# PKU-EPIC/PartManip

Measured on AMD Instinct MI355X. Metric: PPO env-steps/sec (whole node), 4096 envs x 1024-pt clouds, higher is better.
Workload: dtype f32

## Files before the change

### include/partmanip_hip.h

```cpp
#ifndef PARTMANIP_HIP_H
#define PARTMANIP_HIP_H

#include <stddef.h>
#include <stdint.h>

#ifdef __cplusplus
extern "C" {
#endif

#define PM_OK 0
#define PM_EINVAL (-1)
#define PM_EWORKSPACE (-2)
#define PM_EALIGN (-3)
#define PM_EUNSUPPORTED (-4)

#define PM_ACT_NONE 0
#define PM_ACT_TANH 1
#define PM_ACT_RELU 2
#define PM_ACT_LRELU 3
#define PM_ACT_ELU 4
#define PM_ACT_SELU 5
#define PM_ACT_SIGMOID 6
#define PM_ACT_MAX 6

// ... 37 lines not shown
    const float* dY; long lddy; const float* W; long ldw; const float* H; long ldh; float* dX; long lddx; int M, N, K, act;
} pm_linear_bwd_data_desc;
typedef struct pm_linear_bwd_weight_desc {
    const float* dY; long lddy; const float* X; long ldx; float* dW; long lddw; float* db; long slab_stride; int M, N, K;
    int dy_cols, x_cols;
    int pad_;
} pm_linear_bwd_weight_desc;
int pm_linear_fwd_group_f32(int n, const pm_linear_fwd_desc* d, void* stream);
int pm_linear_bwd_data_group_f32(int n, const pm_linear_bwd_data_desc* d, void* stream);
int pm_linear_bwd_weight_group_f32(int n, const pm_linear_bwd_weight_desc* d, int splits, void* stream);
#define PM_LINEAR_PATH_SKINNY 0
#define PM_LINEAR_PATH_REG 1
#define PM_LINEAR_PATH_DMA 2
typedef struct pm_linear_variant {
    int path;
    int tm, tn;
    int lay;
    int stages;
    int vec;
    int big;
    int grid;
    int n;
    int vecC[PM_LINEAR_GROUP_MAX];
    int splits[PM_LINEAR_GROUP_MAX];
    int kchunk[PM_LINEAR_GROUP_MAX];
} pm_linear_variant;
int pm_linear_fwd_variant_f32(const float* X, long ldx, const float* W, long ldw, const float* b, const float* Y, long ldy,
                              int M, int N, int K, int act, pm_linear_variant* out);
int pm_linear_bwd_data_variant_f32(const float* dY, long lddy, const float* W, long ldw, const float* H, long ldh,
                                   const float* dX, long lddx, int M, int N, int K, int act, pm_linear_variant* out);
int pm_linear_bwd_weight_variant_f32(const float* dY, long lddy, const float* X, long ldx, const float* dW, long lddw,
                                     const float* db, int M, int N, int K, const void* workspace, pm_linear_variant* out);
int pm_linear_fwd_group_variant_f32(int n, const pm_linear_fwd_desc* d, pm_linear_variant* out);
int pm_linear_bwd_data_group_variant_f32(int n, const pm_linear_bwd_data_desc* d, pm_linear_variant* out);
int pm_linear_bwd_weight_group_variant_f32(int n, const pm_linear_bwd_weight_desc* d, int splits, pm_linear_variant* out);
size_t pm_linear_chain_workspace_bytes(int M);
int pm_linear_fwd_chain_f32(int n, const pm_linear_fwd_desc* d, void* workspace, size_t workspace_bytes, void* stream);
int pm_linear_bwd_data_chain_f32(int n, const pm_linear_bwd_data_desc* d, void* workspace, size_t workspace_bytes, void* stream);

size_t pm_pointnet_packed_elems(void);
int pm_pointnet_pack_weights_f32(const float* W2, const float* W3, float* packed, void* stream);
int pm_pointnet_enc_fwd_f32(const float* x, long ldx, int B, int P, int C, int sub_mean, const float* W1,
                            const float* b1, const float* b2, const float* b3, const float* packed,
                            int max_mean, float* feat, long ldf, int32_t* argmax,
                            float* h2_save ,
                            int act ,
                            void* stream);
size_t pm_pointnet_packed_screen_bytes(void);
int pm_pointnet_pack_weights_screen(const float* W3, const float* b3, void* packed, void* stream);
int pm_pointnet_enc_fwd_screen_f32(const float* x, long ldx, int B, int P, int C, int sub_mean, const float* W1,
                                   const float* b1, const float* b2, const float* b3, const float* packed,
                                   const void* packed_screen, int max_mean, float* feat, long ldf, int32_t* argmax,
                                   float* h2_save, unsigned long long* counters, void* stream);
size_t pm_pointnet_packed_bf3_bytes(void);
int pm_pointnet_pack_weights_bf3(const float* W2, const float* W3, void* packed, void* stream);
int pm_pointnet_enc_fwd_bf3(const float* x, long ldx, int B, int P, int C, int sub_mean, const float* W1,
                            const float* b1, const float* b2, const float* b3, const void* packed, int max_mean,
                            float* feat, long ldf, int32_t* argmax, float* h2_save ,
                            void* stream);
size_t pm_pointnet_packed_bf6_bytes(void);
int pm_pointnet_pack_weights_bf6(const float* W2, const float* W3, void* packed, void* stream);
int pm_pointnet_enc_fwd_bf6(const float* x, long ldx, int B, int P, int C, int sub_mean, const float* W1,
                            const float* b1, const float* b2, const float* b3, const void* packed, int max_mean,
                            float* feat, long ldf, int32_t* argmax, float* h2_save ,
                            void* stream);
size_t pm_pointnet_enc_bwd_workspace_bytes(int B, int P, int C);
int pm_pointnet_enc_bwd_f32(const float* x, long ldx, int B, int P, int C, int sub_mean, const float* W1,
                            const float* b1, const float* b2, const float* W3, const float* packed,
                            int max_mean, const float* dfeat, long ldf, const int32_t* argmax, float* dW1,
                            float* db1, float* dW2, float* db2, float* dW3, float* db3,
                            const float* h2_saved ,
                            int act , void* workspace, size_t workspace_bytes, void* stream);
size_t pm_pointnet_packed_bwd_bf6_bytes(void);
int pm_pointnet_pack_weights_bwd_bf6(const float* W2, void* packed, void* stream);
int pm_pointnet_enc_bwd_bf6(const float* x, long ldx, int B, int P, int C, int sub_mean, const float* W1,
                            const float* b1, const float* b2, const float* W3, const float* packed,
                            const void* packed_w2_bf6, int max_mean, const float* dfeat, long ldf, const int32_t* argmax,
                            float* dW1, float* db1, float* dW2, float* db2, float* dW3, float* db3, const float* h2_saved,
                            void* workspace, size_t workspace_bytes, void* stream);

int pm_ppo_actor_loss_fwd_bwd_f32(const float* mu, long ldmu, const float* log_std, const float* actions,
                                  long lda, const float* old_logp, const float* adv, const float* old_mu,
                                  long ldom, const float* old_sigma, long ldos, int B, int A, float max_action,
                                  int act_tanh, float eps_clip, float desired_kl, const double* adv_moments,
                                  double adv_count, float* scal_out, float* dmu, long lddmu, float* dlog_std,
                                  void* workspace, size_t workspace_bytes, void* stream);
size_t pm_ppo_actor_loss_workspace_bytes(int B);
int pm_ppo_actor_head_supported(const float* H, long ldh, const float* W, long ldw, int A, int K, const float* dH, long lddh);
int pm_ppo_actor_head_f32(const float* H, long ldh, const float* W, long ldw, const float* bias, int K, int hidden_act,
                          const float* log_std, const float* actions, long lda, const float* old_logp, const float* adv,
                          const float* old_mu, long ldom, const float* old_sigma, long ldos, int B, int A, float max_action,
                          int act_tanh, float eps_clip, float desired_kl, const double* adv_moments, double adv_count,
                          float* scal_out, float* mu_out, long ldmu, float* dmu, long lddmu, float* dH, long lddh,
                          float* dlog_std, void* workspace, size_t workspace_bytes, unsigned int* counter, void* stream);
int pm_gaussian_logp_f32(const float* mu, long ldmu, const float* log_std, const float* actions, long lda,
                         int B, int A, float max_action, int act_tanh, float* logp, float* entropy,
                         void* stream);

int pm_value_loss_fwd_bwd_f32(const float* V, const float* returns, const float* old_values, int B,
                              int clipped, float eps_clip, const float* clip_mean_extern, float grad_scale,
                              float* scal_out, float* dV, long lddv, void* stream);

size_t pm_value_head_workspace_bytes(void);
int pm_value_head_supported(const float* H, long ldh, const float* W, int K, const float* dH, long lddh);
int pm_value_head_f32(const float* H, long ldh, const float* W, const float* bias, int K, int hidden_act, const float* returns,
                      const float* old_values, int B, int clipped, float eps_clip, const float* clip_mean_extern,
// ... 297 lines not shown
```

### partmanip_amd/_lib.py

```python
import ctypes as C
import os

import torch

HERE = os.path.dirname(os.path.abspath(__file__))
LIB_PATH = os.environ.get("PARTMANIP_HIP_LIB") or os.path.join(HERE, "lib", "libpartmanip_hip.so")

P, I, L, F, D, Z = C.c_void_p, C.c_int, C.c_long, C.c_float, C.c_double, C.c_size_t

SIGNATURES = {
    "pm_version": (I, []),
    "pm_gae_scan_f32": (I, [P, P, P, P, P, P, P, I, I, F, F, I, F, P]),
    "pm_moments_workspace_bytes": (Z, [L]),
    "pm_moments_f64": (I, [P, L, P, P, Z, P]),
    "pm_normalize_apply_f32": (I, [P, L, P, D, F, P]),
    "pm_gather_rows_f32": (I, [P, P, P, L, L, L, L, P]),
    "pm_linear_fwd_f32": (I, [P, L, P, L, P, P, L, I, I, I, I, P]),
    "pm_linear_bwd_data_f32": (I, [P, L, P, L, P, L, P, L, I, I, I, I, P]),
    "pm_linear_bwd_weight_workspace_bytes": (Z, [I, I, I]),
    "pm_linear_bwd_weight_f32": (I, [P, L, P, L, P, L, P, I, I, I, P, Z, P]),
    "pm_linear_fwd_group_f32": (I, [I, P, P]),
    "pm_linear_bwd_data_group_f32": (I, [I, P, P]),
    "pm_linear_chain_workspace_bytes": (C.c_size_t, [I]),
    "pm_linear_fwd_chain_f32": (I, [I, P, P, C.c_size_t, P]),
    "pm_linear_bwd_data_chain_f32": (I, [I, P, P, C.c_size_t, P]),
    "pm_linear_bwd_weight_group_f32": (I, [I, P, I, P]),
    "pm_linear_fwd_variant_f32": (I, [P, L, P, L, P, P, L, I, I, I, I, P]),
    "pm_linear_bwd_data_variant_f32": (I, [P, L, P, L, P, L, P, L, I, I, I, I, P]),
    "pm_linear_bwd_weight_variant_f32": (I, [P, L, P, L, P, L, P, I, I, I, P, P]),
    "pm_linear_fwd_group_variant_f32": (I, [I, P, P]),
    "pm_linear_bwd_data_group_variant_f32": (I, [I, P, P]),
    "pm_linear_bwd_weight_group_variant_f32": (I, [I, P, I, P]),
    "pm_clip_adam_group_f32": (I, [I, P, P]),
    "pm_grad_slab_sum_f32": (I, [P, P, L, L, I, P]),
    "pm_pointnet_packed_elems": (Z, []),
    "pm_pointnet_pack_weights_f32": (I, [P, P, P, P]),
    "pm_pointnet_enc_fwd_f32": (I, [P, L, I, I, I, I, P, P, P, P, P, I, P, L, P, P, I, P]),
    "pm_pointnet_packed_screen_bytes": (Z, []),
    "pm_pointnet_pack_weights_screen": (I, [P, P, P, P]),
    "pm_pointnet_enc_fwd_screen_f32": (I, [P, L, I, I, I, I, P, P, P, P, P, P, I, P, L, P, P, P, P]),
    "pm_pointnet_packed_bf3_bytes": (Z, []),
    "pm_pointnet_pack_weights_bf3": (I, [P, P, P, P]),
    "pm_pointnet_enc_fwd_bf3": (I, [P, L, I, I, I, I, P, P, P, P, P, I, P, L, P, P, P]),
    "pm_pointnet_packed_bf6_bytes": (Z, []),
    "pm_pointnet_pack_weights_bf6": (I, [P, P, P, P]),
    "pm_pointnet_enc_fwd_bf6": (I, [P, L, I, I, I, I, P, P, P, P, P, I, P, L, P, P, P]),
    "pm_pointnet_enc_bwd_workspace_bytes": (Z, [I, I, I]),
    "pm_pointnet_enc_bwd_f32": (I, [P, L, I, I, I, I, P, P, P, P, P, I, P, L, P, P, P, P, P, P, P, P, I, P, Z, P]),
    "pm_pointnet_packed_bwd_bf6_bytes": (Z, []),
    "pm_pointnet_pack_weights_bwd_bf6": (I, [P, P, P]),
    "pm_pointnet_enc_bwd_bf6": (I, [P, L, I, I, I, I, P, P, P, P, P, P, I, P, L, P, P, P, P, P, P, P, P, P, Z, P]),
    "pm_ppo_actor_loss_fwd_bwd_f32": (I, [P, L, P, P, L, P, P, P, L, P, L, I, I, F, I, F, F, P, D, P, P, L, P, P, Z, P]),
    "pm_ppo_actor_loss_workspace_bytes": (Z, [I]),
    "pm_ppo_actor_head_supported": (I, [P, L, P, L, I, I, P, L]),
    "pm_ppo_actor_head_f32": (I, [P, L, P, L, P, I, I, P, P, L, P, P, P, L, P, L, I, I, F, I, F, F, P, D, P, P, L, P, L, P, L, P, P, Z, P, P]),
    "pm_gaussian_logp_f32": (I, [P, L, P, P, L, I, I, F, I, P, P, P]),
    "pm_gaussian_logp_bwd_f32": (I, [P, L, P, P, L, I, I, F, I, P, P, P, L, P, P]),
    "pm_action_activation_bwd_f32": (I, [P, P, P, L, F, I, P]),
    "pm_value_loss_fwd_bwd_f32": (I, [P, P, P, I, I, F, P, F, P, P, L, P]),
    "pm_value_head_workspace_bytes": (Z, []),
    "pm_value_head_supported": (I, [P, L, P, I, P, L]),
    "pm_value_head_f32": (I, [P, L, P, P, I, I, P, P, I, I, F, P, F, P, P, P, L, P, L, P, Z, P, P]),
    "pm_mse_tanh_loss_fwd_bwd_f32": (I, [P, L, P, L, I, I, F, I, F, P, P, L, P]),
    "pm_action_activation_f32": (I, [P, P, L, F, I, P]),
    "pm_clip_adam_workspace_bytes": (Z, [L]),
    "pm_clip_adam_step_f32": (I, [P, P, P, P, L, L, F, D, D, D, D, P, P, P, P, Z, P]),
    "pm_ppo_accumulate_stats_f32": (I, [P, P, I, P]),
    "pm_fps_workspace_bytes": (Z, [I, I]),
    "pm_fps_f32": (I, [P, I, I, I, I, P, P, Z, P]),
    "pm_ball_query_f32": (I, [P, P, I, I, I, F, I, P, P]),
    "pm_group_points_f32": (I, [P, P, I, I, I, I, I, P, P]),
    "pm_group_points_bwd_f32": (I, [P, P, I, I, I, I, I, P, P]),
    "pm_group_concat_f32": (I, [P, P, P, P, I, I, I, I, I, I, P, P]),
    "pm_group_concat_bwd_f32": (I, [P, P, I, I, I, I, I, I, P, P]),
    "pm_maxpool_rows_f32": (I, [P, L, I, I, P, L, P, P]),
    "pm_maxpool_rows_bwd_f32": (I, [P, L, P, L, I, I, P, P, P]),
    "pm_depth_backproject_f32": (I, [P, I, I, I, I, P, F, F, F, F, P, P, P, P]),
    "pm_depth_compact_f32": (I, [P, I, I, P, P, P]),
    "pm_fps_varlen_f32": (I, [P, I, I, I, I, P, I, P, P, Z, P]),
    "pm_fps_varlen_workspace_bytes": (Z, [I, I]),
    "pm_tsdf_select_f32": (I, [P, I, I, F, F, P, P, P]),
    "pm_gaussian_sample_f32": (I, [P, L, P, P, I, I, F, I, P, P, P, P]),
    "pm_rms_update_workspace_bytes": (Z, [I]),
    "pm_rms_update_f32": (I, [P, L, I, I, I, P, P, P, P, Z, P]),
    "pm_rms_normalize_f32": (I, [P, L, I, I, P, P, P, L, P]),
    "pm_rms_moments_f64": (I, [P, L, I, I, P, P, Z, P]),
    "pm_rms_apply_moments_f32": (I, [P, L, I, I, P, P, P, P]),
    "pm_tsdf_sparse_gather_f32": (I, [P, P, P, I, I, I, P, P]),
    "pm_im2col3d_f32": (I, [P, I, I, I, I, I, I, I, I, L, L, L, L, L, P, I, P]),
    "pm_conv3d_c1_supported": (I, [I, I]),
    "pm_conv3d_c1_wgrad_workspace_bytes": (Z, [I]),
    "pm_conv3d_c1_fwd_f32": (I, [P, I, I, I, I, I, I, I, L, L, L, L, P, P, I, I, P, L, P, P]),
    "pm_conv3d_c1_wgrad_f32": (I, [P, L, P, I, I, I, I, I, I, I, L, L, L, L, I, P, L, P, P, P, Z, P]),
# ... 139 lines not shown
```

### partmanip_amd/algo_utils/network.py

```python
import math
from typing import NamedTuple, Optional

import torch
import torch.nn as nn

from .. import ops

_LINEAR_ACT = {"tanh": ops.ACT_TANH, "relu": ops.ACT_RELU, "crelu": ops.ACT_RELU, "lrelu": ops.ACT_LRELU, "elu": ops.ACT_ELU,
               "selu": ops.ACT_SELU, "sigmoid": ops.ACT_SIGMOID}
_SUPPORTED_ACT = {"tanh": ops.ACT_TANH}
import os as _os
CHAIN_LAUNCH = _os.environ.get("PARTMANIP_CHAIN", "0") == "1"
PN_SCREEN_DEFAULT = True


def get_activation(act_name):
    table = {"elu": nn.ELU, "selu": nn.SELU, "relu": nn.ReLU, "crelu": nn.ReLU, "lrelu": nn.LeakyReLU,
             "tanh": nn.Tanh, "sigmoid": nn.Sigmoid}
    if act_name not in table:
        print("invalid activation function!")
        return None
    return table[act_name]()


# ... 199 lines not shown
        for g, m in zip(gains, lins):
            torch.nn.init.orthogonal_(m.weight, gain=g)
        object.__setattr__(self, "_chain", _LinearChain(lins, _act_code(net_cfg['activation'], linear_only=True)))

    def set_grad_views(self, views):
        idx = [i for i, m in enumerate(self.model) if isinstance(m, nn.Linear)]
        self._chain.grads = [(views[f"model.{i}.weight"], views[f"model.{i}.bias"]) for i in idx]

    def hip_forward(self, x, out=None, x_w=None):
        return self._chain.forward(x, out, x_w)

    def hip_backward(self, dy):
        self._chain.backward(dy, self._workspace(dy.device))


class PointNet(_HipNet):

    def __init__(self, input_dim, output_dim, net_cfg, proprio_shape):
        super().__init__()
        self.max_mean_concat = net_cfg['max_mean']
        self.point_num = int(net_cfg.get('point_num', 1024))
        act = net_cfg['activation']
        self.mlp = nn.Sequential(
            nn.Linear(input_dim // self.point_num, 128), get_activation(act),
            nn.Linear(128, 256), get_activation(act),
            nn.Linear(256, 512),
        )
        self.final_mlp = nn.Sequential(
            nn.Linear(512 * (1 + self.max_mean_concat) + proprio_shape, 128), get_activation(act),
            nn.Linear(128, 32), get_activation(act),
            nn.Linear(32, output_dim),
        )
        self.proprio_shape = proprio_shape
        self.substract_mean = net_cfg['sub_mean']
        self.count = 0
        self.in_channels = input_dim // self.point_num
        self.feat_dim = 512 * (1 + int(self.max_mean_concat))
        self.precision = net_cfg.get('precision', 'f32')
        self.save_h2 = bool(net_cfg.get('save_h2', True))
        if self.precision not in ('f32', 'bf16x3', 'bf16x6'):
            raise ValueError(f"PointNet precision '{self.precision}'")
        self.precision_bwd = net_cfg.get('precision_bwd', 'f32')
        if self.precision_bwd not in ('f32', 'bf16x6'):
            raise ValueError(f"PointNet precision_bwd '{self.precision_bwd}'")
        if self.precision_bwd != 'f32' and not self.save_h2:
            raise ValueError("PointNet precision_bwd 'bf16x6' reads the forward's saved layer 2 (save_h2: True)")
        code = _act_code(act, linear_only=True)
        if (self.precision != 'f32' or self.precision_bwd != 'f32') and code != ops.ACT_TANH:
            raise NotImplementedError(f"PointNet precision '{self.precision}' / precision_bwd '{self.precision_bwd}' is a tanh "
                                      f"kernel; activation '{act}' runs on 'f32'")
        screen = _os.environ.get("PARTMANIP_PN_SCREEN")
        self.screen = bool(net_cfg.get('screen', PN_SCREEN_DEFAULT)) if screen is None else screen == "1"
        self.screen_counters = None
        object.__setattr__(self, "_act", code)
        object.__setattr__(self, "_packed_s", None)
        object.__setattr__(self, "_head", _LinearChain([self.final_mlp[0], self.final_mlp[2], self.final_mlp[4]], code))
        object.__setattr__(self, "_enc_grads", None)
        object.__setattr__(self, "_packed", None)
        object.__setattr__(self, "_packed3", None)
        object.__setattr__(self, "_packed6", None)
        object.__setattr__(self, "_packed6b", None)

    def set_grad_views(self, views):
        self._head.grads = [(views[f"final_mlp.{i}.weight"], views[f"final_mlp.{i}.bias"]) for i in (0, 2, 4)]
        object.__setattr__(self, "_enc_grads", [views[f"mlp.{i}.{k}"] for i in (0, 2, 4) for k in ("weight", "bias")])

    def _pack(self, device):
        if self._packed is None or self._packed.device != device:
            object.__setattr__(self, "_packed", torch.empty(ops.pointnet_packed_elems(), device=device))
        ops.pointnet_pack(self.mlp[2].weight.data, self.mlp[4].weight.data, self._packed)
        return self._packed

    def forward(self, x):
        with torch.no_grad():
            return self.hip_forward(x, save_h2=False)

    def _h2_buffer(self, B, device):
        return self._scratch("_h2buf", B * self.point_num * 256, device).view(B, self.point_num, 256)

    def hip_forward(self, x, out=None, save_h2=None):
        B = x.shape[0]
        packed = self._pack(x.device)
        feat = torch.empty(B, self.feat_dim + self.proprio_shape, device=x.device)
        argmax = torch.empty(B, 512, dtype=torch.int32, device=x.device)
        save_h2 = self.save_h2 if save_h2 is None else save_h2
        h2 = self._h2_buffer(B, x.device) if save_h2 else None
        if self.precision == 'bf16x3':
            if self._packed3 is None or self._packed3.device != x.device:
                object.__setattr__(self, "_packed3", torch.empty(int(ops.lib.pm_pointnet_packed_bf3_bytes()),
                                                                 dtype=torch.uint8, device=x.device))
            ops.pointnet_pack_bf3(self.mlp[2].weight.data, self.mlp[4].weight.data, self._packed3)
            ops.pointnet_enc_fwd_bf3(x, self.point_num, self.in_channels, self.substract_mean, self.mlp[0].weight.data,
                                     self.mlp[0].bias.data, self.mlp[2].bias.data, self.mlp[4].bias.data,
                                     self._packed3, self.max_mean_concat, feat, argmax, h2)
        elif self.precision == 'bf16x6':
            if self._packed6 is None or self._packed6.device != x.device:
                object.__setattr__(self, "_packed6", torch.empty(int(ops.lib.pm_pointnet_packed_bf6_bytes()),
                                                                 dtype=torch.uint8, device=x.device))
            ops.pointnet_pack_bf6(self.mlp[2].weight.data, self.mlp[4].weight.data, self._packed6)
            ops.pointnet_enc_fwd_bf6(x, self.point_num, self.in_channels, self.substract_mean, self.mlp[0].weight.data,
                                     self.mlp[0].bias.data, self.mlp[2].bias.data, self.mlp[4].bias.data,
                                     self._packed6, self.max_mean_concat, feat, argmax, h2)
        elif self.screen and self._act == ops.ACT_TANH and self.point_num % 64 == 0:
            if self._packed_s is None or self._packed_s.device != x.device:
                object.__setattr__(self, "_packed_s", torch.empty(ops.pointnet_packed_screen_bytes(), dtype=torch.uint8,
                                                                  device=x.device))
            ops.pointnet_pack_screen(self.mlp[4].weight.data, self.mlp[4].bias.data, self._packed_s)
            ops.pointnet_enc_fwd_screen(x, self.point_num, self.in_channels, self.substract_mean, self.mlp[0].weight.data,
                                        self.mlp[0].bias.data, self.mlp[2].bias.data, self.mlp[4].bias.data, packed,
                                        self._packed_s, self.max_mean_concat, feat, argmax, h2, self.screen_counters)
        else:
            ops.pointnet_enc_fwd(x, self.point_num, self.in_channels, self.substract_mean, self.mlp[0].weight.data,
                                 self.mlp[0].bias.data, self.mlp[2].bias.data, self.mlp[4].bias.data, packed,
                                 self.max_mean_concat, feat, argmax, h2, self._act)
        if self.proprio_shape != 0:
            feat[:, self.feat_dim:].copy_(x[:, -self.proprio_shape:])
        object.__setattr__(self, "_saved", (x, feat, argmax, h2))
        return self._head.forward(feat, out)

    def hip_backward(self, dy):
        x, feat, argmax, h2 = self._saved
        ws = self._workspace(dy.device)
        dfeat = torch.empty_like(feat)
        self._head.backward(dy, ws, dx_out=dfeat)
        g = self._enc_grads
        if self.precision_bwd == 'bf16x6':
            if h2 is None:
                raise RuntimeError("PointNet precision_bwd 'bf16x6': the forward did not save layer 2 (an inference forward?)")
            if self._packed6b is None or self._packed6b.device != dy.device:
                object.__setattr__(self, "_packed6b", torch.empty(int(ops.lib.pm_pointnet_packed_bwd_bf6_bytes()),
                                                                  dtype=torch.uint8, device=dy.device))
            ops.pointnet_pack_bwd_bf6(self.mlp[2].weight.data, self._packed6b)
            ops.pointnet_enc_bwd_bf6(x, self.point_num, self.in_channels, self.substract_mean, self.mlp[0].weight.data,
                                     self.mlp[0].bias.data, self.mlp[2].bias.data, self.mlp[4].weight.data, self._packed,
                                     self._packed6b, self.max_mean_concat, dfeat, argmax, g[0], g[1], g[2], g[3], g[4], g[5],
                                     ws, h2)
            return
        ops.pointnet_enc_bwd(x, self.point_num, self.in_channels, self.substract_mean, self.mlp[0].weight.data,
                             self.mlp[0].bias.data, self.mlp[2].bias.data, self.mlp[4].weight.data, self._packed,
                             self.max_mean_concat, dfeat, argmax, g[0], g[1], g[2], g[3], g[4], g[5], ws, h2, self._act)


def _pad4(n):
    return (n + 3) // 4 * 4


class _GeomTabs(list):

    def __init__(self, it=()):
        super().__init__(it)
        self.plans = {}


class _FusedLevel(NamedTuple):
    idx: torch.Tensor
    arg: torch.Tensor
    xyz: torch.Tensor
    feat: Optional[torch.Tensor]
    centers: torch.Tensor
    Y: Optional[torch.Tensor]
    packed: torch.Tensor
    pooled: torch.Tensor
    h2: Optional[torch.Tensor]
# ... 879 lines not shown
```

### partmanip_amd/csrc/pointnet_enc_screen.h

```cpp
#pragma once

typedef __bf16 ps_bf16x8 __attribute__((ext_vector_type(8)));

#define PS_LDP (PN_C2 + 8)
#define PS_CAP 128
#define PS_NW 8
#define PS_P3 (16 * 16 * 64 * 8)
#define PS_OFF_P3H 0
#define PS_OFF_P3L (2 * PS_P3)
#define PS_OFF_W3 (4 * PS_P3 + 8192)
#define PS_OFF_EPS (PS_OFF_W3 + PN_C3 * PN_C2 * 4)
#define PS_PACKED_BYTES (PS_OFF_EPS + PN_C3 * 4)

extern "C" size_t pm_pointnet_packed_screen_bytes(void) { return PS_PACKED_BYTES; }

__device__ __forceinline__ unsigned ps_cvt_pk(float a, float b) {
    unsigned r;
    asm("v_cvt_pk_bf16_f32 %0, %1, %2" : "=v"(r) : "v"(a), "v"(b));
    return r;
}
__device__ __forceinline__ void ps_split(float x, unsigned short& hi, unsigned short& lo) {
    const unsigned h = ps_cvt_pk(x, 0.f) & 0xffffu;
    const float xh = __uint_as_float(h << 16);
    hi = (unsigned short)h;
    lo = (unsigned short)(ps_cvt_pk(x - xh, 0.f) & 0xffffu);
}

__global__ __launch_bounds__(256) void ps_pack_kernel(const float* __restrict__ W3, const float* __restrict__ b3,
                                                       unsigned char* __restrict__ packed) {
    const int i = blockIdx.x * 256 + threadIdx.x;
    if (i >= PS_P3) return;
    unsigned short* Ph = (unsigned short*)(packed + PS_OFF_P3H);
    unsigned short* Pl = (unsigned short*)(packed + PS_OFF_P3L);
    float* Wr = (float*)(packed + PS_OFF_W3);
    const int e = i & 7, lane = (i >> 3) & 63, li = lane & 31, lq = lane >> 5, step = (i >> 9) & 15, nb = i >> 13;
    unsigned short h, l;
    ps_split(W3[(nb * 32 + li) * PN_C2 + step * 16 + lq * 8 + e], h, l);
    Ph[i] = h;
    Pl[i] = l;
    Wr[i] = W3[i];
    if (i < 4096) ((unsigned short*)(packed + 4 * PS_P3))[i] = 0;
    if (i < PN_C3) {
        double L = 0.0;
        for (int k = 0; k < PN_C2; ++k) L += fabs((double)W3[i * PN_C2 + k]);
        const double ed = (0x1p-16 + 2048.0 * 0x1p-24) * (L + fabs((double)b3[i])) * (1.0 + 0x1p-10);
        float ef = (float)ed;
        if ((double)ef < ed) ef = __uint_as_float(__float_as_uint(ef) + 1);
        ((float*)(packed + PS_OFF_EPS))[i] = ef;
    }
}

extern "C" int pm_pointnet_pack_weights_screen(const float* W3, const float* b3, void* packed, void* stream) {
    PM_REQUIRE(W3 && b3 && packed);
    if (((uintptr_t)packed & 15) != 0) return PM_EALIGN;
    hipLaunchKernelGGL(ps_pack_kernel, dim3(PS_P3 / 256), dim3(256), 0, pm_stream(stream), W3, b3, (unsigned char*)packed);
    PM_CHECK_LAUNCH();
    return PM_OK;
}

#define PS_MFMA(a, b, c) __builtin_amdgcn_mfma_f32_32x32x16_bf16((a), (b), (c), 0, 0, 0)
__device__ __forceinline__ ps_bf16x8 ps_bf(const uint4& v) { return *(const ps_bf16x8*)&v; }

__device__ __forceinline__ void ps_stream(const unsigned short* __restrict__ Ah, const unsigned short* __restrict__ Al,
                                          const uint4* __restrict__ Bh, const uint4* __restrict__ Bl, f32x16 (&acc)[2][2]) {
    uint4 bh0[2], bl0[2], bh1[2], bl1[2];
#pragma unroll
    for (int nb = 0; nb < 2; ++nb) {
        bh0[nb] = Bh[(size_t)(nb * 16) * 64];
        bl0[nb] = Bl[(size_t)(nb * 16) * 64];
    }
#define PS_STEP(S_, BHC, BLC, BHN, BLN)                                                        \
    {                                                                                          \
        uint4 ah[2], al[2];                                                                    \
        _Pragma("unroll") for (int mb = 0; mb < 2; ++mb) {                                     \
            ah[mb] = *(const uint4*)(Ah + mb * 32 * PS_LDP + (S_) * 16);                       \
            al[mb] = *(const uint4*)(Al + mb * 32 * PS_LDP + (S_) * 16);                       \
        }                                                                                      \
        _Pragma("unroll") for (int nb = 0; nb < 2; ++nb) {    \
            BHN[nb] = Bh[(size_t)(nb * 16 + (S_) + 1) * 64];                                   \
            BLN[nb] = Bl[(size_t)(nb * 16 + (S_) + 1) * 64];                                   \
        }                                                                                      \
        __builtin_amdgcn_sched_barrier(0);                                                     \
        _Pragma("unroll") for (int nb = 0; nb < 2; ++nb)                                       \
            _Pragma("unroll") for (int mb = 0; mb < 2; ++mb) {                                 \
                acc[mb][nb] = PS_MFMA(ps_bf(ah[mb]), ps_bf(BHC[nb]), acc[mb][nb]);             \
                acc[mb][nb] = PS_MFMA(ps_bf(ah[mb]), ps_bf(BLC[nb]), acc[mb][nb]);             \
                acc[mb][nb] = PS_MFMA(ps_bf(al[mb]), ps_bf(BHC[nb]), acc[mb][nb]);             \
            }                                                                                  \
        __builtin_amdgcn_sched_barrier(0);                                                     \
    }
#pragma unroll 1
    for (int s = 0; s < 16; s += 2) {
        PS_STEP(s, bh0, bl0, bh1, bl1)
        PS_STEP(s + 1, bh1, bl1, bh0, bl0)
    }
#undef PS_STEP
}

template <int CT>
__global__ __launch_bounds__(PS_NW * 64, 2) void pn_fwd_screen_kernel(
    const float* __restrict__ x, long ldx, int P, int C, int sub_mean, const float* __restrict__ W1,
    const float* __restrict__ b1, const float* __restrict__ b2, const float* __restrict__ b3,
    const float* __restrict__ packed, const unsigned char* __restrict__ packed_s, int max_mean, float* __restrict__ feat,
    long ldf, int32_t* __restrict__ argmax, float* __restrict__ h2_save, unsigned long long* __restrict__ counters) {
    constexpr int NT = PS_NW * 64;
    __shared__ __attribute__((aligned(16))) float H[PN_TM * PN_LD2];
    __shared__ __attribute__((aligned(16))) unsigned short Hp[2 * PN_TM * PS_LDP];
    __shared__ __attribute__((aligned(16))) float Xs[PN_TM * PN_MAXC];
    __shared__ double red[16];
    __shared__ double cs[PN_C2];
    __shared__ int skey[PS_NW][PS_CAP];
    __shared__ float sval[PS_NW][PS_CAP];
    unsigned short* Hh = Hp;
    unsigned short* Hl = Hp + PN_TM * PS_LDP;

    const int b = blockIdx.x, tid = threadIdx.x, lane0 = tid & 63, wave = tid >> 6;
    const float* xb = x + (long)b * ldx;
    const float4* P2v = (const float4*)(packed + PN_P2_OFF);
    const float4* P3v = (const float4*)(packed + PN_P3_OFF);
    const uint4* S3h = (const uint4*)(packed_s + PS_OFF_P3H);
    const uint4* S3l = (const uint4*)(packed_s + PS_OFF_P3L);
    const float* W3r = (const float*)(packed_s + PS_OFF_W3);
    const float* epsg = (const float*)(packed_s + PS_OFF_EPS);

    float cen[3] = {0.f, 0.f, 0.f};
    if (sub_mean) cloud_centroid<NT>(xb, P, C, red, cen);

    float vmax = -INFINITY, pois = 0.f;
    int imax = 0;
    double csum = 0.0;

    const int ntiles = P / PN_TM;
    stage_points<PN_TM, NT>(xb, 0, C, sub_mean, cen, Xs);
    for (int tile = 0; tile < ntiles; ++tile) {
        int lane = lane0;
        asm volatile("" : "+v"(lane));
        const int li = lane & 31, lh = lane >> 5;
        __syncthreads();
        layer1_tile<CT, PN_TM, NT, true>(Xs, W1, b1, C, H);
        __syncthreads();
        {
            f32x16 acc2[2][1];
            zero_acc<2, 1>(acc2);
            layer2_mfma<2, 1>(H, P2v, wave, lane, acc2);
            __syncthreads();
            const int col = wave * 32 + li;
            const float b2c = b2[col];
            float ts = 0.f;
#pragma unroll
            for (int mb = 0; mb < 2; ++mb)
#pragma unroll
                for (int r = 0; r < 16; r += 2) {
                    const f32x2 v2 = pm_tanh2(acc2[mb][0][r] + b2c, acc2[mb][0][r + 1] + b2c);
#pragma unroll
                    for (int j = 0; j < 2; ++j) {
                        const int row = mb * 32 + ((r + j) & 3) + 8 * ((r + j) >> 2) + 4 * lh;
                        const float v = j ? v2.y : v2.x;
                        unsigned short hi, lo;
                        ps_split(v, hi, lo);
                        H[row * PN_LD2 + col] = v;
                        Hh[row * PS_LDP + col] = hi;
                        Hl[row * PS_LDP + col] = lo;
                        ts += v;
                    }
                }
            ts += __shfl_xor(ts, 32, 64);
            csum += (double)ts;
            if (tile + 1 < ntiles) stage_points<PN_TM, NT>(xb, tile + 1, C, sub_mean, cen, Xs);
        }
        __syncthreads();

        f32x16 acc[2][2];
#pragma unroll
        for (int nb = 0; nb < 2; ++nb) {
            const float b3c = b3[(wave * 2 + nb) * 32 + li];
#pragma unroll
            for (int r = 0; r < 16; ++r) acc[0][nb][r] = acc[1][nb][r] = b3c;
        }
        ps_stream(Hh + li * PS_LDP + lh * 8, Hl + li * PS_LDP + lh * 8, S3h + (size_t)(wave * 2 * 16) * 64 + lane,
                  S3l + (size_t)(wave * 2 * 16) * 64 + lane, acc);

        unsigned msk[2];
#pragma unroll
        for (int nb = 0; nb < 2; ++nb) {
            float m = -INFINITY;
#pragma unroll
            for (int mb = 0; mb < 2; ++mb)
#pragma unroll
                for (int r = 0; r < 16; ++r) m = fmaxf(m, acc[mb][nb][r]);
            m = fmaxf(m, __shfl_xor(m, 32, 64));
            const float e = epsg[(wave * 2 + nb) * 32 + li];
            const float vm = __shfl(vmax, nb * 32 + li, 64);
            const float thr = m - 2.f * e;
            unsigned k = 0;
#pragma unroll
            for (int mb = 0; mb < 2; ++mb)
#pragma unroll
                for (int r = 0; r < 16; ++r) {
                    const float z = acc[mb][nb][r];
                    const bool s = !(z < thr) && !(z + e <= vm);
                    k |= (s ? 1u : 0u) << (mb * 16 + r);
                }
            msk[nb] = k;
        }
        const int n = __popc(msk[0]) + __popc(msk[1]);
        int incl = n;
#pragma unroll
        for (int o = 1; o < 64; o <<= 1) {
            const int t = __shfl_up(incl, o, 64);
            if (lane >= o) incl += t;
        }
        const int total = __builtin_amdgcn_readlane(incl, 63);

        if (total <= PS_CAP) {
            int off = incl - n;
#pragma unroll
            for (int nb = 0; nb < 2; ++nb) {
                unsigned m = msk[nb];
                while (m) {
                    const int bit = __ffs(m) - 1;
                    m &= m - 1;
                    const int row = (bit >> 4) * 32 + (bit & 3) + 8 * ((bit & 15) >> 2) + 4 * lh;
                    skey[wave][off++] = (row << 6) | (nb * 32 + li);
                }
            }
            __builtin_amdgcn_wave_barrier();
            const int j = lane & 7, g = lane >> 3;
            for (int e0 = 0; e0 < total; e0 += 8) {
                const int e = e0 + g;
                const int key = (e < total) ? skey[wave][e] : 0;
                const int row = key >> 6, cl = key & 63;
                const float* hp = H + row * PN_LD2 + 4 * j;
                const float* wp = W3r + (size_t)(wave * 64 + cl) * PN_C2 + 4 * j;
                float s = 0.f;
#pragma unroll
                for (int i = 0; i < 8; ++i) {
                    const float4 w = *(const float4*)(wp + 32 * i);
                    const float4 h = *(const float4*)(hp + 32 * i);
                    s = fmaf(w.x, h.x, s);
                    s = fmaf(w.y, h.y, s);
                    s = fmaf(w.z, h.z, s);
                    s = fmaf(w.w, h.w, s);
                }
                s += __shfl_xor(s, 4, 64);
                s += __shfl_xor(s, 2, 64);
                s += __shfl_xor(s, 1, 64);
                s += b3[wave * 64 + cl];
                if (j == 0 && e < total) sval[wave][e] = s;
            }
            __builtin_amdgcn_wave_barrier();
            for (int e = 0; e < total; ++e) {
                const int key = skey[wave][e];
                const float v = sval[wave][e];
                if ((key & 63) == lane) {
                    const int p = tile * PN_TM + (key >> 6);
                    if (!(fabsf(v) < INFINITY)) pois += v;
                    if (v > vmax || (v == vmax && p < imax)) {
                        vmax = v;
                        imax = p;
                    }
                }
            }
            if (counters) {
                const unsigned long long h0 = __ballot(msk[0] != 0), h1 = __ballot(msk[1] != 0);
                if (lane == 0) {
                    atomicAdd(counters + 0, (unsigned long long)total);
                    atomicAdd(counters + 2, (unsigned long long)(__popc((unsigned)(h0 | (h0 >> 32))) + __popc((unsigned)(h1 | (h1 >> 32)))));
                }
            }
        } else {
#pragma unroll
            for (int nb = 0; nb < 2; ++nb) {
                const float b3c = b3[(wave * 2 + nb) * 32 + li];
#pragma unroll
                for (int r = 0; r < 16; ++r) acc[0][nb][r] = acc[1][nb][r] = b3c;
            }
            mfma_stream<2, 2, 32>(H + li * PN_LD2 + lh * 128, PN_LD2, P3v + (size_t)(wave * 2) * 32 * 64 + lane, acc);
#pragma unroll
            for (int nb = 0; nb < 2; ++nb) {
                float bv = -INFINITY, ps = 0.f;
                int bp = 0;
#pragma unroll
                for (int mb = 0; mb < 2; ++mb)
#pragma unroll
                    for (int r = 0; r < 16; ++r) {
                        const float v = acc[mb][nb][r];
                        if (!(fabsf(v) < INFINITY)) ps += v;
                        if (v > bv) {
                            bv = v;
                            bp = tile * PN_TM + mb * 32 + (r & 3) + 8 * (r >> 2) + 4 * lh;
                        }
                    }
                const float ov = __shfl_xor(bv, 32, 64), os = __shfl_xor(ps, 32, 64);
                const int op = __shfl_xor(bp, 32, 64);
                if (ov > bv || (ov == bv && op < bp)) {
                    bv = ov;
                    bp = op;
                }
                if (lh == nb) {
                    pois += ps + os;
                    if (bv > vmax || (bv == vmax && bp < imax)) {
                        vmax = bv;
                        imax = bp;
                    }
                }
            }
            if (counters && lane == 0) atomicAdd(counters + 1, 1ull);
        }
        if (h2_save) {
            float* dst = h2_save + ((long)b * P + (long)tile * PN_TM) * PN_C2;
#pragma unroll 2
            for (int i = 0; i < PN_TM * PN_C2 / 4 / NT; ++i) {
                const int q = tid + NT * i, row = q >> 6, c4 = q & 63;
                const f32x4 v = *(const f32x4*)(H + row * PN_LD2 + 4 * c4);
                *(f32x4*)(dst + row * PN_C2 + 4 * c4) = v;
            }
        }
    }
    if ((lane0 >> 5) == 0) cs[wave * 32 + lane0] = csum;
    __syncthreads();
    const int ch = tid;
    float v = vmax;
    if (pois != pois) v = pois;
    feat[(long)b * ldf + ch] = v;
    argmax[(long)b * PN_C3 + ch] = imax;
    if (max_mean) {
        const float* wr = W3r + (size_t)ch * PN_C2;
        double s = 0.0;
#pragma unroll 4
        for (int k = 0; k < PN_C2; k += 4) {
            const float4 w = *(const float4*)(wr + k);
            s = fma((double)w.x, cs[k], s);
            s = fma((double)w.y, cs[k + 1], s);
            s = fma((double)w.z, cs[k + 2], s);
            s = fma((double)w.w, cs[k + 3], s);
        }
        float mv = (float)(s / (double)P + (double)b3[ch]);
        if (pois != pois) mv = pois;
        feat[(long)b * ldf + PN_C3 + ch] = mv;
    }
}

extern "C" int pm_pointnet_enc_fwd_screen_f32(const float* x, long ldx, int B, int P, int C, int sub_mean, const float* W1,
                                              const float* b1, const float* b2, const float* b3, const float* packed,
                                              const void* packed_screen, int max_mean, float* feat, long ldf,
                                              int32_t* argmax, float* h2_save, unsigned long long* counters, void* stream) {
    PM_REQUIRE(x && W1 && b1 && b2 && b3 && packed && packed_screen && feat && argmax);
    if (h2_save && ((uintptr_t)h2_save & 15) != 0) return PM_EALIGN;
    PM_REQUIRE(B > 0 && P > 0 && P % PN_TM == 0 && C >= 1 && C <= PN_MAXC && ldx >= (long)P * C);
    PM_REQUIRE(ldf >= PN_C3 * (max_mean ? 2 : 1));
    PM_REQUIRE(!sub_mean || C >= 3);
    if (((uintptr_t)packed & 15) != 0 || ((uintptr_t)packed_screen & 15) != 0 || ((uintptr_t)counters & 7) != 0) return PM_EALIGN;
#define PS_LAUNCH(CT)                                                                                                 \
    hipLaunchKernelGGL((pn_fwd_screen_kernel<CT>), dim3(B), dim3(PS_NW * 64), 0, pm_stream(stream), x, ldx, P, C, sub_mean, \
                       W1, b1, b2, b3, packed, (const unsigned char*)packed_screen, max_mean, feat, ldf, argmax, h2_save,   \
                       counters)
    if (C == 3) PS_LAUNCH(3);
    else if (C == 4) PS_LAUNCH(4);
    else PS_LAUNCH(0);
#undef PS_LAUNCH
    PM_CHECK_LAUNCH();
    return PM_OK;
}
```

### partmanip_amd/ops.py

```python
import ctypes as C
import os

import torch

from ._lib import lib, check

ACT_NONE, ACT_TANH, ACT_RELU, ACT_LRELU, ACT_ELU, ACT_SELU, ACT_SIGMOID = range(7)


def _ptr(t):
    return 0 if t is None else t.data_ptr()


class KernelTimer:

    def __init__(self):
        self.enabled = set()
        self.events = {}

    def enable(self, *names):
        self.enabled = set(names)
        self.events = {n: [] for n in names}

    def add(self, *names):
# ... 339 lines not shown
        _req(p, g, it["m"], it["v"], it["state"], it.get("skip_flag"), it.get("gnorm"), it.get("extra"))
        n = p.numel()
        w = it["ws"].get(lib.pm_clip_adam_workspace_bytes(n) + 8)
        base = w.data_ptr()
        d.params, d.grads, d.exp_avg, d.exp_avg_sq, d.n, d.n_clip = _ptr(p), _ptr(g), _ptr(it["m"]), _ptr(it["v"]), n, int(it["n_clip"])
        d.extra, d.extra_stride, d.n_sum, d.n_extra = _ptr(it.get("extra")), int(it.get("extra_stride", 0)), int(it.get("n_sum", 0)), int(it.get("n_extra", 0))
        d.max_norm, d.lr, d.b1, d.b2, d.eps = float(it["max_norm"]), float(it["lr"]), float(it["b1"]), float(it["b2"]), float(it["eps"])
        d.state, d.skip_flag, d.gnorm_out, d.workspace = _ptr(it["state"]), _ptr(it.get("skip_flag")), _ptr(it.get("gnorm")), base + (-base) % 8
        dp = it.get("dp")
        if dp is not None:
            _req(dp[1])
            d.grad_scale, d.dp_scal, d.dp_kl_desired = float(dp[0]), _ptr(dp[1]), float(dp[2])
        st = it.get("stats")
        if st is not None:
            _req(st[0], st[1])
            d.stats_acc, d.stats_scal, d.stats_which = _ptr(st[0]), _ptr(st[1]), int(st[2])
    check(lib.pm_clip_adam_group_f32(len(items), arr, _stream()), "pm_clip_adam_group_f32")


def grad_slab_sum(g, extra, extra_stride, n_sum, n_extra):
    _req(g, extra)
    check(lib.pm_grad_slab_sum_f32(_ptr(g), _ptr(extra), int(extra_stride), int(n_sum), int(n_extra), _stream()), "pm_grad_slab_sum_f32")


def pointnet_packed_elems():
    return int(lib.pm_pointnet_packed_elems())


def pointnet_pack(w2, w3, packed):
    _req(w2, w3, packed)
    check(lib.pm_pointnet_pack_weights_f32(_ptr(w2), _ptr(w3), _ptr(packed), _stream()), "pm_pointnet_pack_weights_f32")


def pointnet_enc_fwd(x, P, Cc, sub_mean, w1, b1, b2, b3, packed, max_mean, feat, argmax, h2_save=None, act=None):
    _req(x, w1, b1, b2, b3, packed, feat, argmax, h2_save)
    B = x.shape[0]
    with TIMER.bracket("pointnet_enc_fwd"):
        check(lib.pm_pointnet_enc_fwd_f32(_ptr(x), _rows(x, "x"), B, P, Cc, int(sub_mean), _ptr(w1), _ptr(b1), _ptr(b2),
                                          _ptr(b3), _ptr(packed), int(max_mean), _ptr(feat), _rows(feat, "feat"),
                                          _ptr(argmax), _ptr(h2_save), int(ACT_TANH if act is None else act), _stream()),
              "pm_pointnet_enc_fwd_f32")


def pointnet_packed_screen_bytes():
    return int(lib.pm_pointnet_packed_screen_bytes())


def pointnet_pack_screen(w3, b3, packed):
    _req(w3, b3, packed)
    check(lib.pm_pointnet_pack_weights_screen(_ptr(w3), _ptr(b3), _ptr(packed), _stream()), "pm_pointnet_pack_weights_screen")


def pointnet_enc_fwd_screen(x, P, Cc, sub_mean, w1, b1, b2, b3, packed, packed_screen, max_mean, feat, argmax, h2_save=None,
                            counters=None):
    _req(x, w1, b1, b2, b3, packed, packed_screen, feat, argmax, h2_save, counters)
    if counters is not None and (counters.dtype != torch.int64 or counters.numel() < 3 or not counters.is_contiguous()):
        raise ValueError("counters: expected a contiguous int64 tensor of 3 elements")
    B = x.shape[0]
    with TIMER.bracket("pointnet_enc_fwd"):
        check(lib.pm_pointnet_enc_fwd_screen_f32(_ptr(x), _rows(x, "x"), B, P, Cc, int(sub_mean), _ptr(w1), _ptr(b1), _ptr(b2),
                                                 _ptr(b3), _ptr(packed), _ptr(packed_screen), int(max_mean), _ptr(feat),
                                                 _rows(feat, "feat"), _ptr(argmax), _ptr(h2_save), _ptr(counters), _stream()),
              "pm_pointnet_enc_fwd_screen_f32")


def pointnet_pack_bf3(w2, w3, packed):
    _req(w2, w3, packed)
    check(lib.pm_pointnet_pack_weights_bf3(_ptr(w2), _ptr(w3), _ptr(packed), _stream()), "pm_pointnet_pack_weights_bf3")


def pointnet_enc_fwd_bf3(x, P, Cc, sub_mean, w1, b1, b2, b3, packed, max_mean, feat, argmax, h2_save=None):
    _req(x, w1, b1, b2, b3, packed, feat, argmax)
    B = x.shape[0]
    with TIMER.bracket("pointnet_enc_fwd"):
        check(lib.pm_pointnet_enc_fwd_bf3(_ptr(x), _rows(x, "x"), B, P, Cc, int(sub_mean), _ptr(w1), _ptr(b1), _ptr(b2),
                                          _ptr(b3), _ptr(packed), int(max_mean), _ptr(feat), _rows(feat, "feat"),
                                          _ptr(argmax), _ptr(h2_save), _stream()), "pm_pointnet_enc_fwd_bf3")


def pointnet_pack_bf6(w2, w3, packed):
    _req(w2, w3, packed)
    check(lib.pm_pointnet_pack_weights_bf6(_ptr(w2), _ptr(w3), _ptr(packed), _stream()), "pm_pointnet_pack_weights_bf6")


def pointnet_enc_fwd_bf6(x, P, Cc, sub_mean, w1, b1, b2, b3, packed, max_mean, feat, argmax, h2_save=None):
    _req(x, w1, b1, b2, b3, packed, feat, argmax)
    B = x.shape[0]
    with TIMER.bracket("pointnet_enc_fwd"):
        check(lib.pm_pointnet_enc_fwd_bf6(_ptr(x), _rows(x, "x"), B, P, Cc, int(sub_mean), _ptr(w1), _ptr(b1), _ptr(b2),
                                          _ptr(b3), _ptr(packed), int(max_mean), _ptr(feat), _rows(feat, "feat"),
                                          _ptr(argmax), _ptr(h2_save), _stream()), "pm_pointnet_enc_fwd_bf6")


def pointnet_enc_bwd(x, P, Cc, sub_mean, w1, b1, b2, w3, packed, max_mean, dfeat, argmax, dw1, db1, dw2, db2, dw3, db3,
                     ws, h2_saved=None, act=None):
    _req(x, w1, b1, b2, w3, packed, dfeat, argmax, dw1, db1, dw2, db2, dw3, db3, h2_saved)
    B = x.shape[0]
    w = ws.get(lib.pm_pointnet_enc_bwd_workspace_bytes(B, P, Cc) + 256)
    base = w.data_ptr()
    al = (-base) % 256
    with TIMER.bracket("pointnet_enc_bwd"):
        check(lib.pm_pointnet_enc_bwd_f32(_ptr(x), _rows(x, "x"), B, P, Cc, int(sub_mean), _ptr(w1), _ptr(b1), _ptr(b2),
                                          _ptr(w3), _ptr(packed), int(max_mean), _ptr(dfeat), _rows(dfeat, "dfeat"),
                                          _ptr(argmax), _ptr(dw1), _ptr(db1), _ptr(dw2), _ptr(db2), _ptr(dw3),
                                          _ptr(db3), _ptr(h2_saved), int(ACT_TANH if act is None else act), base + al,
                                          w.numel() - al, _stream()),
              "pm_pointnet_enc_bwd_f32")


def pointnet_pack_bwd_bf6(w2, packed):
    _req(w2, packed)
# ... 1472 lines not shown
```

Before: 32190.

## Pack bf16 split planes via DPP, drop sval LDS, add staggered h2 copy schedule

```diff
diff --git a/include/partmanip_hip.h b/include/partmanip_hip.h
--- a/include/partmanip_hip.h
+++ b/include/partmanip_hip.h
@@ -113,6 +113,10 @@
                                    const float* b1, const float* b2, const float* b3, const float* packed,
                                    const void* packed_screen, int max_mean, float* feat, long ldf, int32_t* argmax,
                                    float* h2_save, unsigned long long* counters, void* stream);
+int pm_pointnet_enc_fwd_screen_sched_f32(const float* x, long ldx, int B, int P, int C, int sub_mean, const float* W1,
+                                         const float* b1, const float* b2, const float* b3, const float* packed,
+                                         const void* packed_screen, int max_mean, float* feat, long ldf, int32_t* argmax,
+                                         float* h2_save, unsigned long long* counters, int schedule, void* stream);
 size_t pm_pointnet_packed_bf3_bytes(void);
 int pm_pointnet_pack_weights_bf3(const float* W2, const float* W3, void* packed, void* stream);
 int pm_pointnet_enc_fwd_bf3(const float* x, long ldx, int B, int P, int C, int sub_mean, const float* W1,
diff --git a/partmanip_amd/_lib.py b/partmanip_amd/_lib.py
--- a/partmanip_amd/_lib.py
+++ b/partmanip_amd/_lib.py
@@ -39,6 +39,7 @@
     "pm_pointnet_packed_screen_bytes": (Z, []),
     "pm_pointnet_pack_weights_screen": (I, [P, P, P, P]),
     "pm_pointnet_enc_fwd_screen_f32": (I, [P, L, I, I, I, I, P, P, P, P, P, P, I, P, L, P, P, P, P]),
+    "pm_pointnet_enc_fwd_screen_sched_f32": (I, [P, L, I, I, I, I, P, P, P, P, P, P, I, P, L, P, P, P, I, P]),
     "pm_pointnet_packed_bf3_bytes": (Z, []),
     "pm_pointnet_pack_weights_bf3": (I, [P, P, P, P]),
     "pm_pointnet_enc_fwd_bf3": (I, [P, L, I, I, I, I, P, P, P, P, P, I, P, L, P, P, P]),
diff --git a/partmanip_amd/algo_utils/network.py b/partmanip_amd/algo_utils/network.py
--- a/partmanip_amd/algo_utils/network.py
+++ b/partmanip_amd/algo_utils/network.py
@@ -275,6 +275,8 @@
         screen = _os.environ.get("PARTMANIP_PN_SCREEN")
         self.screen = bool(net_cfg.get('screen', PN_SCREEN_DEFAULT)) if screen is None else screen == "1"
         self.screen_counters = None
+        stagger = _os.environ.get("PARTMANIP_PN_SCREEN_STAGGER")
+        self.screen_schedule = None if stagger is None else int(stagger)
         object.__setattr__(self, "_act", code)
         object.__setattr__(self, "_packed_s", None)
         object.__setattr__(self, "_head", _LinearChain([self.final_mlp[0], self.final_mlp[2], self.final_mlp[4]], code))
@@ -331,7 +333,8 @@
             ops.pointnet_pack_screen(self.mlp[4].weight.data, self.mlp[4].bias.data, self._packed_s)
             ops.pointnet_enc_fwd_screen(x, self.point_num, self.in_channels, self.substract_mean, self.mlp[0].weight.data,
                                         self.mlp[0].bias.data, self.mlp[2].bias.data, self.mlp[4].bias.data, packed,
-                                        self._packed_s, self.max_mean_concat, feat, argmax, h2, self.screen_counters)
+                                        self._packed_s, self.max_mean_concat, feat, argmax, h2, self.screen_counters,
+                                        self.screen_schedule)
         else:
             ops.pointnet_enc_fwd(x, self.point_num, self.in_channels, self.substract_mean, self.mlp[0].weight.data,
                                  self.mlp[0].bias.data, self.mlp[2].bias.data, self.mlp[4].bias.data, packed,
diff --git a/partmanip_amd/csrc/pointnet_enc_screen.h b/partmanip_amd/csrc/pointnet_enc_screen.h
--- a/partmanip_amd/csrc/pointnet_enc_screen.h
+++ b/partmanip_amd/csrc/pointnet_enc_screen.h
@@ -11,6 +11,12 @@
 #define PS_OFF_W3 (4 * PS_P3 + 8192)
 #define PS_OFF_EPS (PS_OFF_W3 + PN_C3 * PN_C2 * 4)
 #define PS_PACKED_BYTES (PS_OFF_EPS + PN_C3 * 4)
+#ifndef PS_ABLATE
+#define PS_ABLATE 0
+#endif
+#ifndef PS_SCHED_DEFAULT
+#define PS_SCHED_DEFAULT 0
+#endif
 
 extern "C" size_t pm_pointnet_packed_screen_bytes(void) { return PS_PACKED_BYTES; }
 
@@ -97,7 +103,20 @@
 #undef PS_STEP
 }
 
-template <int CT>
+template <int SCHED>
+__device__ __forceinline__ bool ps_late_wave(int wave) { return SCHED == 1 && __builtin_amdgcn_readfirstlane(wave) >= 4; }
+
+template <int NT>
+__device__ __forceinline__ void ps_copy_h2(const float* __restrict__ H, float* __restrict__ dst, int tid) {
+#pragma unroll 2
+    for (int i = 0; i < PN_TM * PN_C2 / 4 / NT; ++i) {
+        const int q = tid + NT * i, row = q >> 6, c4 = q & 63;
+        const f32x4 v = *(const f32x4*)(H + row * PN_LD2 + 4 * c4);
+        *(f32x4*)(dst + row * PN_C2 + 4 * c4) = v;
+    }
+}
+
+template <int CT, int SCHED>
 __global__ __launch_bounds__(PS_NW * 64, 2) void pn_fwd_screen_kernel(
     const float* __restrict__ x, long ldx, int P, int C, int sub_mean, const float* __restrict__ W1,
     const float* __restrict__ b1, const float* __restrict__ b2, const float* __restrict__ b3,
@@ -110,7 +129,6 @@
     __shared__ double red[16];
     __shared__ double cs[PN_C2];
     __shared__ int skey[PS_NW][PS_CAP];
-    __shared__ float sval[PS_NW][PS_CAP];
     unsigned short* Hh = Hp;
     unsigned short* Hl = Hp + PN_TM * PS_LDP;
 
@@ -137,31 +155,59 @@
         asm volatile("" : "+v"(lane));
         const int li = lane & 31, lh = lane >> 5;
         __syncthreads();
-        layer1_tile<CT, PN_TM, NT, true>(Xs, W1, b1, C, H);
+        if (!(PS_ABLATE & 1)) layer1_tile<CT, PN_TM, NT, true>(Xs, W1, b1, C, H);
         __syncthreads();
         {
             f32x16 acc2[2][1];
             zero_acc<2, 1>(acc2);
-            layer2_mfma<2, 1>(H, P2v, wave, lane, acc2);
+            if (PS_ABLATE & 2) {
+#pragma unroll
+                for (int mb = 0; mb < 2; ++mb)
+#pragma unroll
+                    for (int r = 0; r < 16; ++r)
+                        acc2[mb][0][r] = H[(mb * 32 + (r & 3) + 8 * (r >> 2) + 4 * lh) * PN_LD1 + ((wave * 32 + li) & 127)];
+            } else {
+                layer2_mfma<2, 1>(H, P2v, wave, lane, acc2);
+            }
             __syncthreads();
             const int col = wave * 32 + li;
             const float b2c = b2[col];
             float ts = 0.f;
+            const bool planes = !(PS_ABLATE & 8) || tile == 0;
+            const bool odd = (lane & 1) != 0;
+            unsigned* Hh2 = (unsigned*)(Hh + (odd ? PS_LDP : 0) + (col & ~1));
+            unsigned* Hl2 = (unsigned*)(Hl + (odd ? PS_LDP : 0) + (col & ~1));
 #pragma unroll
             for (int mb = 0; mb < 2; ++mb)
 #pragma unroll
                 for (int r = 0; r < 16; r += 2) {
-                    const f32x2 v2 = pm_tanh2(acc2[mb][0][r] + b2c, acc2[mb][0][r + 1] + b2c);
-#pragma unroll
-                    for (int j = 0; j < 2; ++j) {
-                        const int row = mb * 32 + ((r + j) & 3) + 8 * ((r + j) >> 2) + 4 * lh;
-                        const float v = j ? v2.y : v2.x;
-                        unsigned short hi, lo;
-                        ps_split(v, hi, lo);
-                        H[row * PN_LD2 + col] = v;
-                        Hh[row * PS_LDP + col] = hi;
-                        Hl[row * PS_LDP + col] = lo;
-                        ts += v;
+                    const float z0 = acc2[mb][0][r] + b2c, z1 = acc2[mb][0][r + 1] + b2c;
+                    f32x2 v2;
+                    if (PS_ABLATE & 4) {
+                        v2.x = z0;
+                        v2.y = z1;
+                    } else {
+                        v2 = pm_tanh2(z0, z1);
+                    }
+                    const int row0 = mb * 32 + (r & 3) + 8 * (r >> 2) + 4 * lh;
+                    H[row0 * PN_LD2 + col] = v2.x;
+                    H[(row0 + 1) * PN_LD2 + col] = v2.y;
+                    ts += v2.x;
+                    ts += v2.y;
+                    const float own = odd ? v2.y : v2.x, send = odd ? v2.x : v2.y;
+                    const float recv = __int_as_float(__builtin_amdgcn_update_dpp(0, __float_as_int(send), 0xB1, 0xf, 0xf, false));
+                    const float a = odd ? recv : own, c = odd ? own : recv;
+                    unsigned h2w, l2w;
+                    if (PS_ABLATE & 4) {
+                        h2w = (__float_as_uint(a) >> 16) | (__float_as_uint(c) & 0xffff0000u);
+                        l2w = 0;
+                    } else {
+                        h2w = ps_cvt_pk(a, c);
+                        l2w = ps_cvt_pk(a - __uint_as_float(h2w << 16), c - __uint_as_float(h2w & 0xffff0000u));
+                    }
+                    if (planes) {
+                        Hh2[row0 * (PS_LDP / 2)] = h2w;
+                        Hl2[row0 * (PS_LDP / 2)] = l2w;
                     }
                 }
             ts += __shfl_xor(ts, 32, 64);
@@ -170,6 +216,10 @@
         }
         __syncthreads();
 
+        const bool copy = h2_save && !(PS_ABLATE & 128), late = ps_late_wave<SCHED>(wave);
+        float* h2dst = copy ? h2_save + ((long)b * P + (long)tile * PN_TM) * PN_C2 : nullptr;
+        if (copy && late) ps_copy_h2<NT>(H, h2dst, tid);
+
         f32x16 acc[2][2];
 #pragma unroll
         for (int nb = 0; nb < 2; ++nb) {
@@ -177,10 +227,30 @@
 #pragma unroll
             for (int r = 0; r < 16; ++r) acc[0][nb][r] = acc[1][nb][r] = b3c;
         }
-        ps_stream(Hh + li * PS_LDP + lh * 8, Hl + li * PS_LDP + lh * 8, S3h + (size_t)(wave * 2 * 16) * 64 + lane,
-                  S3l + (size_t)(wave * 2 * 16) * 64 + lane, acc);
+        if (PS_ABLATE & 16) {
+#pragma unroll
+            for (int nb = 0; nb < 2; ++nb)
+#pragma unroll
+                for (int mb = 0; mb < 2; ++mb)
+#pragma unroll
+                    for (int r = 0; r < 16; ++r)
+                        acc[mb][nb][r] += H[(mb * 32 + (r & 3) + 8 * (r >> 2) + 4 * lh) * PN_LD2 + ((wave * 64 + nb * 32 + li) & 255)];
+        } else {
+            ps_stream(Hh + li * PS_LDP + lh * 8, Hl + li * PS_LDP + lh * 8, S3h + (size_t)(wave * 2 * 16) * 64 + lane,
+                      S3l + (size_t)(wave * 2 * 16) * 64 + lane, acc);
+        }
 
         unsigned msk[2];
+        float tmax[2];
+#if (PS_ABLATE & 32) && defined(__HIP_DEVICE_COMPILE__)
+#pragma unroll
+        for (int nb = 0; nb < 2; ++nb) {
+#pragma unroll
+            for (int mb = 0; mb < 2; ++mb) asm volatile("" ::"v"(acc[mb][nb]));
+            msk[nb] = 0;
+            tmax[nb] = 0.f;
+        }
+#else
 #pragma unroll
         for (int nb = 0; nb < 2; ++nb) {
             float m = -INFINITY;
@@ -202,7 +272,9 @@
                     k |= (s ? 1u : 0u) << (mb * 16 + r);
                 }
             msk[nb] = k;
-        }
+            tmax[nb] = m;
+        }
+#endif
         const int n = __popc(msk[0]) + __popc(msk[1]);
         int incl = n;
 #pragma unroll
@@ -212,7 +284,10 @@
         }
         const int total = __builtin_amdgcn_readlane(incl, 63);
 
-        if (total <= PS_CAP) {
+        if (PS_ABLATE & 64) {
+            vmax = fmaxf(vmax, lh ? tmax[1] : tmax[0]);
+            if (counters && lane == 0) atomicAdd(counters + 0, (unsigned long long)total);
+        } else if (total <= PS_CAP) {
             int off = incl - n;
 #pragma unroll
             for (int nb = 0; nb < 2; ++nb) {
@@ -246,20 +321,20 @@
                 s += __shfl_xor(s, 2, 64);
                 s += __shfl_xor(s, 1, 64);
                 s += b3[wave * 64 + cl];
-                if (j == 0 && e < total) sval[wave][e] = s;
-            }
-            __builtin_amdgcn_wave_barrier();
-            for (int e = 0; e < total; ++e) {
-                const int key = skey[wave][e];
-                const float v = sval[wave][e];
-                if ((key & 63) == lane) {
-                    const int p = tile * PN_TM + (key >> 6);
-                    if (!(fabsf(v) < INFINITY)) pois += v;
-                    if (v > vmax || (v == vmax && p < imax)) {
-                        vmax = v;
-                        imax = p;
-                    }
-                }
+#pragma unroll
+                for (int gg = 0; gg < 8; ++gg)
+                    if (e0 + gg < total) {
+                        const int kk = __builtin_amdgcn_readlane(key, gg * 8);
+                        const float v = __int_as_float(__builtin_amdgcn_readlane(__float_as_int(s), gg * 8));
+                        if ((kk & 63) == lane) {
+                            const int p = tile * PN_TM + (kk >> 6);
+                            if (!(fabsf(v) < INFINITY)) pois += v;
+                            if (v > vmax || (v == vmax && p < imax)) {
+                                vmax = v;
+                                imax = p;
+                            }
+                        }
+                    }
             }
             if (counters) {
                 const unsigned long long h0 = __ballot(msk[0] != 0), h1 = __ballot(msk[1] != 0);
@@ -307,15 +382,7 @@
             }
             if (counters && lane == 0) atomicAdd(counters + 1, 1ull);
         }
-        if (h2_save) {
-            float* dst = h2_save + ((long)b * P + (long)tile * PN_TM) * PN_C2;
-#pragma unroll 2
-            for (int i = 0; i < PN_TM * PN_C2 / 4 / NT; ++i) {
-                const int q = tid + NT * i, row = q >> 6, c4 = q & 63;
-                const f32x4 v = *(const f32x4*)(H + row * PN_LD2 + 4 * c4);
-                *(f32x4*)(dst + row * PN_C2 + 4 * c4) = v;
-            }
-        }
+        if (copy && !late) ps_copy_h2<NT>(H, h2dst, tid);
     }
     if ((lane0 >> 5) == 0) cs[wave * 32 + lane0] = csum;
     __syncthreads();
@@ -341,24 +408,40 @@
     }
 }
 
-extern "C" int pm_pointnet_enc_fwd_screen_f32(const float* x, long ldx, int B, int P, int C, int sub_mean, const float* W1,
-                                              const float* b1, const float* b2, const float* b3, const float* packed,
-                                              const void* packed_screen, int max_mean, float* feat, long ldf,
-                                              int32_t* argmax, float* h2_save, unsigned long long* counters, void* stream) {
+extern "C" int pm_pointnet_enc_fwd_screen_sched_f32(const float* x, long ldx, int B, int P, int C, int sub_mean, const float* W1,
+                                                    const float* b1, const float* b2, const float* b3, const float* packed,
+                                                    const void* packed_screen, int max_mean, float* feat, long ldf,
+                                                    int32_t* argmax, float* h2_save, unsigned long long* counters, int schedule,
+                                                    void* stream) {
     PM_REQUIRE(x && W1 && b1 && b2 && b3 && packed && packed_screen && feat && argmax);
+    PM_REQUIRE(schedule == 0 || schedule == 1);
     if (h2_save && ((uintptr_t)h2_save & 15) != 0) return PM_EALIGN;
     PM_REQUIRE(B > 0 && P > 0 && P % PN_TM == 0 && C >= 1 && C <= PN_MAXC && ldx >= (long)P * C);
     PM_REQUIRE(ldf >= PN_C3 * (max_mean ? 2 : 1));
     PM_REQUIRE(!sub_mean || C >= 3);
     if (((uintptr_t)packed & 15) != 0 || ((uintptr_t)packed_screen & 15) != 0 || ((uintptr_t)counters & 7) != 0) return PM_EALIGN;
-#define PS_LAUNCH(CT)                                                                                                 \
-    hipLaunchKernelGGL((pn_fwd_screen_kernel<CT>), dim3(B), dim3(PS_NW * 64), 0, pm_stream(stream), x, ldx, P, C, sub_mean, \
+#define PS_LAUNCH(CT, S)                                                                                              \
+    hipLaunchKernelGGL((pn_fwd_screen_kernel<CT, S>), dim3(B), dim3(PS_NW * 64), 0, pm_stream(stream), x, ldx, P, C, sub_mean, \
                        W1, b1, b2, b3, packed, (const unsigned char*)packed_screen, max_mean, feat, ldf, argmax, h2_save,   \
                        counters)
-    if (C == 3) PS_LAUNCH(3);
-    else if (C == 4) PS_LAUNCH(4);
-    else PS_LAUNCH(0);
+    if (schedule == 0) {
+        if (C == 3) PS_LAUNCH(3, 0);
+        else if (C == 4) PS_LAUNCH(4, 0);
+        else PS_LAUNCH(0, 0);
+    } else {
+        if (C == 3) PS_LAUNCH(3, 1);
+        else if (C == 4) PS_LAUNCH(4, 1);
+        else PS_LAUNCH(0, 1);
+    }
 #undef PS_LAUNCH
     PM_CHECK_LAUNCH();
     return PM_OK;
 }
+
+extern "C" int pm_pointnet_enc_fwd_screen_f32(const float* x, long ldx, int B, int P, int C, int sub_mean, const float* W1,
+                                              const float* b1, const float* b2, const float* b3, const float* packed,
+                                              const void* packed_screen, int max_mean, float* feat, long ldf,
+                                              int32_t* argmax, float* h2_save, unsigned long long* counters, void* stream) {
+    return pm_pointnet_enc_fwd_screen_sched_f32(x, ldx, B, P, C, sub_mean, W1, b1, b2, b3, packed, packed_screen, max_mean, feat,
+                                                ldf, argmax, h2_save, counters, PS_SCHED_DEFAULT, stream);
+}
diff --git a/partmanip_amd/ops.py b/partmanip_amd/ops.py
--- a/partmanip_amd/ops.py
+++ b/partmanip_amd/ops.py
@@ -415,11 +415,19 @@
 
 
 def pointnet_enc_fwd_screen(x, P, Cc, sub_mean, w1, b1, b2, b3, packed, packed_screen, max_mean, feat, argmax, h2_save=None,
-                            counters=None):
+                            counters=None, schedule=None):
     _req(x, w1, b1, b2, b3, packed, packed_screen, feat, argmax, h2_save, counters)
     if counters is not None and (counters.dtype != torch.int64 or counters.numel() < 3 or not counters.is_contiguous()):
         raise ValueError("counters: expected a contiguous int64 tensor of 3 elements")
     B = x.shape[0]
+    if schedule is not None:
+        with TIMER.bracket("pointnet_enc_fwd"):
+            check(lib.pm_pointnet_enc_fwd_screen_sched_f32(_ptr(x), _rows(x, "x"), B, P, Cc, int(sub_mean), _ptr(w1), _ptr(b1),
+                                                           _ptr(b2), _ptr(b3), _ptr(packed), _ptr(packed_screen), int(max_mean),
+                                                           _ptr(feat), _rows(feat, "feat"), _ptr(argmax), _ptr(h2_save),
+                                                           _ptr(counters), int(schedule), _stream()),
+                  "pm_pointnet_enc_fwd_screen_sched_f32")
+        return
     with TIMER.bracket("pointnet_enc_fwd"):
         check(lib.pm_pointnet_enc_fwd_screen_f32(_ptr(x), _rows(x, "x"), B, P, Cc, int(sub_mean), _ptr(w1), _ptr(b1), _ptr(b2),
                                                  _ptr(b3), _ptr(packed), _ptr(packed_screen), int(max_mean), _ptr(feat),
```

New measurement: 32640, median of 6. 1.4% higher.
